# lukeshope/hipims-ocl

Hardware: AMD Instinct MI355X
Metric: Mcell-steps/sec fp64 Godunov+HLLC, 4096^2 grid, 1/2/4/8 MI355X; % HBM roofline (higher is better)
Workload: dtype f64

## Files before the change

hipims-ocl_amd/csrc/hp_engine.hip:

```cpp
#include "hp_domain.hpp"
#include "hp_observers.hpp"
#include "hp_actors.hpp"
#include <hip/hip_ext.h>
#include <dlfcn.h>

#include <algorithm>
#include <cmath>
#include <cstdio>
#include <cstdlib>
#include <cstring>
#include <random>
#include <string>
#include <vector>
#include <unistd.h>

namespace {

constexpr size_t CFL_SLOT_BYTES = 1024;

struct Rccl {
	void* handle = nullptr;
	decltype(&ncclGetUniqueId)   GetUniqueId = nullptr;
	decltype(&ncclCommInitRank)  CommInitRank = nullptr;
	decltype(&ncclCommDestroy)   CommDestroy = nullptr;
// ... 2 lines not shown
	decltype(&ncclSend)          Send = nullptr;
	decltype(&ncclRecv)          Recv = nullptr;
	decltype(&ncclAllReduce)     AllReduce = nullptr;
	decltype(&ncclGetErrorString) GetErrorString = nullptr;
	decltype(&ncclCommCount)     CommCount = nullptr;
	std::string path;
} g_rccl;

void peer_release(hp_domain* d);
PeerBox peer_box(hp_domain* d, bool use, long timeout_ms = 0);
PeerPush make_push(const hp_domain* d);

const PlanKnobs& plan_knobs()
{
	static const PlanKnobs knobs = [] {
		auto num = [](const char* name, int unset) { const char* e = std::getenv(name); return e ? std::atoi(e) : unset; };
		auto off = [&](const char* name) { return num(name, 1) == 0; };
		auto on = [&](const char* name) { return num(name, 0) != 0; };
		auto force = [&](const char* name) { return std::getenv(name) ? (num(name, 0) != 0 ? 1 : 0) : -1; };
		PlanKnobs k;
		k.two_step = num("HP_TWO_STEP", -1);
		k.launch_tail = !off("HP_LAUNCH_TAIL"); k.strip_reduce_always = on("HP_STRIP_REDUCE_ALWAYS");
		k.pair_bdy = !off("HP_PAIR_BDY"); k.pair_strict = !off("HP_PAIR_STRICT"); k.pair_exact = force("HP_PAIR_EXACT");
		k.pair_skip = !off("HP_PAIR_SKIP"); k.fill_after_pairs = !off("HP_FILL_AFTER_PAIRS");
		k.strict_speculate = on("HP_STRICT_SPECULATE"); k.pair_tune = !off("HP_PAIR_TUNE"); k.sweep_alternate = force("HP_SWEEP_ALTERNATE");
		k.tail_max_blocks = (unsigned)num("HP_TAIL_MAX_BLOCKS", (int)TAIL_MAX_BLOCKS);
		k.tail_max_blocks_k2k6 = (unsigned)num("HP_TAIL_MAX_BLOCKS_K2K6", (int)TAIL_MAX_BLOCKS);
		k.march2_rseg_forced = std::getenv("HP_MARCH2_RSEG") != nullptr;
		k.fuse_bdy = !off("HP_FUSE_BDY");
		return k;
	}();
	return knobs;
}
PlanDomain plan_domain(const hp_domain* d)
{
	PlanDomain p;
	p.scheme = d->desc.scheme; p.kernel = d->desc.kernel; p.math_mode = d->desc.math_mode; p.precision = d->desc.precision; p.dynamic_dt = d->desc.dynamic_dt;
	p.quirks = d->desc.quirks; p.rows = d->desc.rows; p.cols = d->desc.cols; p.cells = d->cells;
	p.row_offset = d->desc.row_offset; p.global_rows = d->desc.global_rows; p.ghost_rows = d->ghost_rows;
	p.has_bdy = !d->bdy.empty(); p.fusable = d->fusable; p.bdy_on_ring = d->bdy_on_ring;
	for (const Boundary& b : d->bdy)
		if ((b.kind == BDY_UNIFORM && b.definition == HP_UNIFORM_LOSS_RATE) || (b.kind == BDY_GRIDDED && b.definition == HP_GRIDDED_MASS_FLUX)) p.bdy_removes_water = true;
	p.has_comm = d->comm != nullptr; p.comm_world = d->comm_world; p.peer_direct = d->peer_direct; p.peer_mine = d->peer_mine != nullptr;
	p.has_tail_words = d->tail_words != nullptr; p.tail_allowed = d->tail_allowed; p.halo_overlap = d->halo_overlap; p.split_now = d->split_now;
	p.strip_any_bdy = d->strip_any_bdy; p.strip_first = d->strip_first; p.strip_any_full = d->strip_any_full;
	p.spec_now = d->spec_now; p.has_stamps = d->z_state != nullptr; p.march2_pays = d->tiling.march2_pays;
	p.has_links = d->links.groups != 0; p.soil_on = d->soil.on; p.tracer_on = d->tracer.on;
// ... 533 lines not shown
	bool in_place = false;
	if (bdy && !d->facts->m1_valid) {
		if ((rc = pair_cold_start<T>(d)) != HP_OK) return rc;
		in_place = true;
	} else if (bdy) in_place = d->facts->pair_fused_next;
	tail.pair = bdy ? 2 : 1;
	tail.bdy_flag = bdy && followed ? 1 : 0;
	PairAux<T> aux{};
	const bool exact = pair_exact(pd, knobs) && d->z_state != nullptr;
	if (exact) aux.stamps = StampBufs<T>{(char*)d->z_state, d->haz_words};
	aux.prev_gen = d->facts->other_stale ? d->pair_gen : 0u;
	aux.gen = ++d->pair_gen;
	if (aux.gen == 0) aux.gen = ++d->pair_gen;
	aux.list = (const AreaBdyList<T>*)d->fused_list; aux.fuse_next = bdy && followed ? 1 : 0; aux.in_place = in_place ? 1 : 0;
	aux.truncated = (d->desc.quirks & HP_QUIRK_BDY_TRUNCATED) != 0 ? 1 : 0;
	const bool recs = pair_records(pd, knobs, strip, exact, rseg2);
	if (recs) {
		if ((rc = still_rec_alloc(d, tm.nstrips)) != HP_OK) return rc;
		StillRec* const base = (StillRec*)d->still_rec;
		aux.still_out = base + (size_t)(d->still_rec_half ^ 1) * d->still_rec_slots;
		aux.still_in = d->facts->still_rec_valid ? base + (size_t)d->still_rec_half * d->still_rec_slots : nullptr;
		aux.still_rows = d->desc.rows;
	}
	const bool ordered = pair_order_on() && d->desc.precision == 8 && d->desc.math_mode != HP_MATH_STRICT && !strip && !bdy && !exact &&
	                     tm.groups <= (int)ORDER_MAX_GROUPS;
	bool order_read = false;
	if (ordered) {
		if ((rc = order_alloc(d, tm)) != HP_OK) return rc;
		order_read = d->order_written && d->flux_launches == d->order_launch + 1;
		const size_t table = (size_t)tm.nbands * tm.groups * (tm.nbig + tm.ntail);
		aux.order_in = order_read ? d->order_buf + (size_t)d->order_half * table : nullptr;
		aux.order_out = d->order_buf + (size_t)(d->order_half ^ 1) * table;
		aux.order_flags = d->order_buf + 2 * table;
	}
	const void* src = d->state[0];
	void* dst = d->state[1];
	const bool sample = d->timing_stride > 0 && d->timing_used < d->timing_events.size() &&
	                    (d->timing_counter++ % (uint64_t)d->timing_stride) == 0;
	if (sample) HIP_TRY(hipEventRecord(d->timing_events[d->timing_used].first, d->stream));
#define HP_LAUNCH_K1B2(CFL_, BDY_, HZ_, TAIL_)                                                                                            \
	hipLaunchKernelGGL((godunov_march2<false, CFL_, BDY_, HZ_, TAIL_, T>), dim3(blocks), dim3(256), 0, d->stream, p, (const Scalars<T>*)d->scalars, \
	                   (const T*)d->bed, (const State4<T>*)src, (State4<T>*)dst, (const T*)d->manning, (T*)d->cfl_slot,                    \
	                   (const T*)d->cfl_slot + SLOT_EDGE, tm, tail, aux)
#define HP_LAUNCH_K1B(CFL_, BDY_, TAIL_) do { if (exact) HP_LAUNCH_K1B2(CFL_, BDY_, true, TAIL_); else HP_LAUNCH_K1B2(CFL_, BDY_, false, TAIL_); } while (0)
	if (d->desc.math_mode == HP_MATH_STRICT)
		hipLaunchKernelGGL((godunov_march2<true, 1, false, true, 1, T>), dim3(blocks), dim3(256), 0, d->stream, p, (const Scalars<T>*)d->scalars,
// ... 1335 lines not shown
	d->timing_stride = enable_stride > 0 ? enable_stride : 0;
	return HP_OK;
}

int hp_kernel_timing_read(hp_domain_t* d, double* avg_ms, uint32_t* samples)
{
	int rc = check_domain(d);
	if (rc != HP_OK) return rc;
	if (!avg_ms || !samples) return fail(HP_ERR_INVALID, "null argument");
	HIP_TRY(hipStreamSynchronize(d->stream));
	double total = 0.0;
	uint32_t n = 0;
	for (size_t i = 0; i < d->timing_used; ++i) {
		float ms = 0.f;
		HIP_TRY(hipEventElapsedTime(&ms, d->timing_events[i].first, d->timing_events[i].second));
		total += std::max(0.0, (double)ms - d->timing_overhead_ms);
		++n;
	}
	*avg_ms = n ? total / n : 0.0;
	*samples = n;
	return HP_OK;
}

int hp_pair_stats(hp_domain_t* d, uint64_t out[12])
{
	int rc = check_domain(d);
	if (rc != HP_OK) return rc;
	if (!out) return fail(HP_ERR_INVALID, "out == NULL");
	out[0] = d->pairs; out[1] = d->pair_cold_starts; out[2] = out[3] = 0;
	HIP_TRY(hipStreamSynchronize(d->stream));
	if (tuner_on(plan_domain(d), plan_knobs()) && (rc = tuner_poll(d)) != HP_OK) return rc;
	out[4] = d->tune_samples; out[5] = d->tune_switches; out[6] = d->tune_prefer_pairs ? 1 : 0;
	out[7] = d->tune_single_ms > 0.f ? (uint64_t)(1000.0 * d->tune_pair_ms / d->tune_single_ms) : 0;
	out[8] = out[9] = out[10] = out[11] = 0;
	if (d->still_rec && d->still_rec_last) {
		const StillRec* half = (const StillRec*)d->still_rec + (size_t)d->still_rec_half * d->still_rec_slots;
		unsigned long long* counts = (unsigned long long*)((StillRec*)d->still_rec + 2 * d->still_rec_slots);
		HIP_TRY(hipMemsetAsync(counts, 0, 16, d->stream));
		hipLaunchKernelGGL(still_rec_count, dim3(256), dim3(256), 0, d->stream, half, d->still_rec_slots, counts);
		HIP_TRY(hipGetLastError());
		unsigned long long host_counts[2] = {0, 0};
		HIP_TRY(hipMemcpyAsync(host_counts, counts, sizeof host_counts, hipMemcpyDeviceToHost, d->stream));
		HIP_TRY(hipStreamSynchronize(d->stream));
		out[9] = host_counts[0]; out[10] = host_counts[1];
	}
	if (d->order_buf && d->order_read) {
		const unsigned per_band = (unsigned)(d->order_shape[1] * (d->order_shape[2] + d->order_shape[3])), table = (unsigned)d->order_shape[0] * per_band;
		unsigned* const count = d->order_buf + 2 * (size_t)table + (size_t)d->order_shape[0] * d->order_shape[1];
		HIP_TRY(hipMemsetAsync(count, 0, sizeof(unsigned), d->stream));
		hipLaunchKernelGGL(order_count, dim3(16), dim3(256), 0, d->stream, d->order_buf + (size_t)(d->order_half ^ 1) * table, (unsigned)d->order_shape[1],
		                   per_band, table, count);
		HIP_TRY(hipGetLastError());
		unsigned moved = 0;
		HIP_TRY(hipMemcpyAsync(&moved, count, sizeof moved, hipMemcpyDeviceToHost, d->stream));
		HIP_TRY(hipStreamSynchronize(d->stream));
		out[11] = moved;
	}
	if (d->haz_words) {
		unsigned long long used = 0;
		HIP_TRY(hipMemcpy(&used, d->haz_words + 2, sizeof used, hipMemcpyDeviceToHost));
		out[8] = used;
	}
	if (!d->z_state) return HP_OK;
	unsigned long long* counts = d->haz_words + 4;
	HIP_TRY(hipMemsetAsync(counts, 0, 16, d->stream));
	if (d->desc.precision == 8)
// ... 32 lines not shown
```

hipims-ocl_amd/csrc/hp_kernels.hpp:

```cpp
#pragma once

#include "hp_math.hpp"
#include "hp_tiling.hpp"
#include "hp_order.hpp"

namespace hp {

template <bool STRICT, typename T>
__global__ __launch_bounds__(256) void godunov_basic(const Params<T> p, const Scalars<T>* __restrict__ sc,
                                                     const T* __restrict__ bed, const State4<T>* __restrict__ src,
                                                     State4<T>* __restrict__ dst, const T* __restrict__ manning,
                                                     const long y_lo, const long y_hi)
{
	const long x = (long)blockIdx.x * blockDim.x + threadIdx.x;
	const long y = (long)blockIdx.y * blockDim.y + threadIdx.y + y_lo;
	if (x >= p.cols - 1 || y >= y_hi || x <= 0) return;
	const size_t id = (size_t)y * p.cols + x;
	const T dt = sc->dt;

	if (dt <= T(0)) { dst[id] = src[id]; return; }

	const State4<T> c = src[id];
	const T zb = bed[id], n = manning[id];
	if (c.zmax <= T(-9999.0) || c.z == T(-9999.0)) { dst[id] = c; return; }
// ... 509 lines not shown
template <typename T> struct AreaBdyList { int count; AreaBdy<T> b[AREA_BDY_MAX]; };


constexpr int FUSED_BDY_MAX = 3;
template <typename T> struct FusedBdy {
	T    inc_lo, inc_hi;
	int  y_switch;
	int  mode;
};

template <typename T> constexpr unsigned stamp_rec() { return (unsigned)sizeof(State4<T>) + 16u; }
template <typename T> struct StampBufs { char* rec; unsigned long long* haz; };
template <typename T> __device__ __forceinline__ unsigned stamp_gen(const StampBufs<T>& b, const size_t id)
{
	return *reinterpret_cast<const unsigned*>(b.rec + id * stamp_rec<T>() + sizeof(State4<T>));
}
template <typename T> __device__ __forceinline__ State4<T> stamp_state(const StampBufs<T>& b, const size_t id)
{
	const T* v = reinterpret_cast<const T*>(b.rec + id * stamp_rec<T>());
	State4<T> c; c.z = v[0]; c.zmax = v[1]; c.qx = v[2]; c.qy = v[3];
	return c;
}
struct StillRec { unsigned long long z, b; unsigned tag, pad[3]; };
constexpr unsigned STILL_TAG_RUN = 1, STILL_TAG_SKIP = 2;
template <typename T> struct PairAux {
	StampBufs<T>          stamps;
	unsigned              gen, prev_gen;
	const AreaBdyList<T>* list;
	int                   fuse_next;
	int                   in_place;
	int                   truncated;
	StillRec*             still_out;
	const StillRec*       still_in;
	long                  still_rows;
	const unsigned*       order_in;
	unsigned*             order_out;
	unsigned*             order_flags;
};

#ifndef HP_K1_STRICT_WAVES
#define HP_K1_STRICT_WAVES 3
#endif
#ifndef HP_K1_FAST_WAVES
#define HP_K1_FAST_WAVES 3
#endif
#ifndef HP_K1_F32_WAVES
#define HP_K1_F32_WAVES 5
#endif
template <bool STRICT, typename T> constexpr int march_waves() { return sizeof(T) == 4 ? HP_K1_F32_WAVES : (STRICT ? HP_K1_STRICT_WAVES : HP_K1_FAST_WAVES); }

template <bool STRICT, typename T> constexpr int march_waves_max() { return sizeof(T) == 4 ? 8 : march_waves<STRICT, T>(); }
template <bool STRICT, int CFL_MODE, bool FUSED, int TAIL, typename T, bool SPEC = false>
__global__ __launch_bounds__(256) __attribute__((amdgpu_waves_per_eu(march_waves<STRICT, T>(), march_waves_max<STRICT, T>()))) void godunov_march(const Params<T> p, const Scalars<T>* sc,
                                                     const T* __restrict__ bed, const State4<T>* __restrict__ src,
                                                     State4<T>* __restrict__ dst, const T* __restrict__ manning,
                                                     T* cfl_slot, const T* __restrict__ edge_max,
                                                     const TileMap tm, const AreaBdyList<T>* __restrict__ fused_list,
// ... 489 lines not shown
	}
	const bool fuse = BDY && aux.fuse_next != 0;

	T vmax = T(0), vmax1 = T(0);
	unsigned stale_rows = 0;

	constexpr bool RECS = !STRICT && !BDY && !HZ && TAIL == 1 && sizeof(T) == 8;
	unsigned long long still_kz = 0, still_kb = 0;
	unsigned still_marks = 0;
	auto write_recs = [&](const unsigned tag) {
		if (!RECS || aux.still_out == nullptr) return;
		const __amdgpu_buffer_rsrc_t srd = make_srd(aux.still_out + (size_t)strip * aux.still_rows, (size_t)aux.still_rows * sizeof(StillRec));
		const bool m = lane < 32 && ((still_marks >> (unsigned)lane) & 1u) != 0;
		hp_u32x4 a;
		a.x = m ? (unsigned)still_kz : ~0u; a.y = m ? (unsigned)(still_kz >> 32) : ~0u;
		a.z = m ? (unsigned)still_kb : ~0u; a.w = m ? (unsigned)(still_kb >> 32) : ~0u;
		unsigned voff = lane < y1 - y0 ? (unsigned)((y0 + lane) * (long)sizeof(StillRec)) : HP_OOB;
		asm volatile("" : "+v"(voff));
		store_operands_own(a);
		__builtin_amdgcn_raw_buffer_store_b128(a, srd, (int)voff, 0, 0);
		__builtin_amdgcn_raw_buffer_store_b32(m ? tag : 0u, srd, (int)voff + 16, 0, 0);
		store_fence(a, voff, 0u);
	};
	auto tile_known = [&]() -> bool {
		const long xw = strip * MARCH2_COLS - 1;
		if (xw < 1 || xw + 63 > p.cols - 2 || y0 - 2 < 1 || y1 + 1 > last_row - 1 || y1 - y0 > 32) return false;
		const int nr = (int)(y1 - y0) + 4, n = 3 * nr;
		const __amdgpu_buffer_rsrc_t srd = make_srd(aux.still_in + (size_t)(strip - 1) * aux.still_rows, (size_t)3 * aux.still_rows * sizeof(StillRec));
		auto voff = [&](const int i) {
			const int w = i < nr ? 0 : (i < 2 * nr ? 1 : 2);
			return i < n ? (unsigned)(((long)w * aux.still_rows + y0 - 2 + (i - w * nr)) * (long)sizeof(StillRec)) : HP_OOB;
		};
		const hp_u32x4 e0 = __builtin_amdgcn_raw_buffer_load_b128(srd, (int)voff(lane), 0, 0);
		const hp_u32x4 e1 = __builtin_amdgcn_raw_buffer_load_b128(srd, (int)voff(lane + 64), 0, 0);
		const unsigned k0 = __builtin_amdgcn_readfirstlane(e0.x), k1 = __builtin_amdgcn_readfirstlane(e0.y);
		const unsigned k2 = __builtin_amdgcn_readfirstlane(e0.z), k3 = __builtin_amdgcn_readfirstlane(e0.w);
		if (k0 == ~0u && k1 == ~0u) return false;
		auto same = [&](const hp_u32x4& e) { return e.x == k0 && e.y == k1 && e.z == k2 && e.w == k3; };
		if (!wave_all((lane >= n || same(e0)) && (lane + 64 >= n || same(e1)))) return false;
		still_kz = ((unsigned long long)k1 << 32) | k0;
		still_kb = ((unsigned long long)k3 << 32) | k2;
		return true;
	};

	auto march = [&](auto live_tag, auto look_tag) {
	constexpr bool LIVE = decltype(live_tag)::value;
	constexpr bool LOOK = decltype(look_tag)::value;
	auto apply = [&](auto j_tag, State4<T> c, const T zb, const long y) {
// ... 220 lines not shown
		rP = load_row(yb);
		{
			RowRegs<T> rs = load_row(yb - 2);
			if (live0) { rs.c = apply(J0(), rs.c, rs.zb, yb - 2 < 0 ? 0 : yb - 2); rc.c = apply(J0(), rc.c, rc.zb, yb - 1); }
			const Side<T> sS = make_side<STRICT>(rs.c.z, rs.c.qx, rs.c.qy, rs.zb, vs);
			sCa = make_side<STRICT>(rc.c.z, rc.c.qx, rc.c.qy, rc.zb, vs);
			drySa = (rs.c.z - rs.zb) < vs;
			if (STILL) {
				if (at_rest(rs.c)) stA |= REST_S;
				if (at_rest(rc.c)) stA |= REST_C;
				if (stA == (REST_S | REST_C) && same_level(rs.c, rs.zb, rc.c, rc.zb)) stA |= EQ_S;
			}
			if (!skip_a) fSa = face_solve<AXIS_Y, STRICT, true, true>(sS, sCa, vs).forR;
		}
		const T n0 = rc.n;
		uc = stage_a(yb - 1, rP, rQ);
		n_c = n0;
		sCb = make_side<STRICT>(uc.c.z, uc.c.qx, uc.c.qy, uc.zb, vs);
		if (STILL && at_rest(uc.c)) stB |= REST_C;
		const T n1 = rc.n;
		const RowU1<T> u0 = stage_a(yb, rQ, rP);
		stage_b(yb - 1, u0, n1, false);
	};
	auto still_run = [&]() -> long {
		auto load_rz = [&](const long yl) {
			unsigned vs_ = yl <= y1 + 1 ? voff_state : HP_OOB, vc_ = yl <= y1 + 1 ? voff_scalar : HP_OOB;
			asm volatile("" : "+v"(vs_), "+v"(vc_));
			const unsigned k = (unsigned)((yl < 0 ? 0 : (yl > last_row ? last_row : yl)) - row_base);
			RowRegs<T> q;
			q.c = buf_load_state(srd_src, vs_, k * row_state, T());
			q.zb = buf_load_scalar(srd_bed, vc_, k * row_scalar, T());
			return q;
		};
		long y = y0;
		RowRegs<T> q[4];
		#pragma unroll
		for (int j = 0; j < 4; ++j) q[j] = load_rz(y - 2 + j);
		const T z0 = first_lane(q[0].c.z), b0 = first_lane(q[0].zb), h0 = z0 - b0;
		if (!(h0 > vs && h0 < T(1e100) && z0 != T(-9999.0))) return y;
		const unsigned long long run_z = value_bits(z0), run_b = value_bits(b0);
		auto in_run = [&](const RowRegs<T>& q_) {
			return wave_all(value_bits(q_.c.z) == run_z && value_bits(q_.zb) == run_b && value_bits(q_.c.qx) == 0 && value_bits(q_.c.qy) == 0 &&
			                !(q_.c.zmax <= T(-9999.0))) != 0;
		};
		if (!(in_run(q[0]) && in_run(q[1]) && in_run(q[2]) && in_run(q[3]))) return y;
		const T spd = cfl_speed<STRICT>(q[2].c.z, q[2].c.zmax, q[2].c.qx, q[2].c.qy, q[2].zb, p.qs);
		still_kz = run_z; still_kb = run_b;
		auto put = [&](State4<T> c, const long yy) {
			if (RECS && !wave_any(!(c.zmax > T(-9999.0)) || (c.z > c.zmax && c.zmax > T(-9990.0)))) still_marks |= 1u << (unsigned)(yy - y0);
			if (c.z > c.zmax && c.zmax > T(-9990.0)) c.zmax = c.z;
			const unsigned row_k = (unsigned)__builtin_amdgcn_readfirstlane((int)(yy - row_base));
			buf_store_state(c, srd_dst, out_x ? voff_state : HP_OOB, row_k * row_state);
			if (TAIL == 2) store_peer(c, yy, out_x);
			if (CFL_MODE == 1 && out_x && (int)yy >= tm.price_lo && (int)yy < tm.price_hi && spd > vmax) vmax = spd;
		};
		State4<T> a = q[2].c, b = q[3].c;
		for (;;) {
			if (y >= y1) return y;
			#pragma unroll
			for (int j = 0; j < 4; ++j) q[j] = load_rz(y + 2 + j);
			if (!in_run(q[0])) return y;
			put(a, y);
			if (y + 1 >= y1 || !in_run(q[1])) return y + 1;
			put(b, y + 1);
			if (y + 2 >= y1 || !in_run(q[2])) return y + 2;
			put(q[0].c, y + 2);
			if (y + 3 >= y1 || !in_run(q[3])) return y + 3;
			put(q[1].c, y + 3);
			a = q[2].c; b = q[3].c;
			y += 4;
		}
	};

	const long yb = (RUNS && !skip_a && !skip_b) ? still_run() : y0;
	write_recs(STILL_TAG_RUN);
	if (!RUNS || yb < y1) {
		if constexpr (ORDERED) { if (order_word != nullptr && lane == 0) __hip_atomic_fetch_add(order_word, 1u, __ATOMIC_RELAXED, __HIP_MEMORY_SCOPE_AGENT); }
		prime(yb);
		long r = yb + 1;
		for (; r + 1 <= y1; r += 2) {
			{ const T nn = rc.n; const RowU1<T> u = stage_a(r, rP, rQ); stage_b(r - 1, u, nn, true); }
			{ const T nn = rc.n; const RowU1<T> u = stage_a(r + 1, rQ, rP); stage_b(r, u, nn, true); }
		}
		if (r <= y1) { const T nn = rc.n; const RowU1<T> u = stage_a(r, rP, rQ); stage_b(r - 1, u, nn, true); }
	}

	if (wave_any(stale_rows != 0)) {
		for (long y = y0; y < y1; ++y) {
			if ((stale_rows >> (unsigned)(y - y0)) & 1u) {
				const size_t id = (size_t)y * p.cols + xc;
				const T zb = bed[id];
				State4<T> c = src[id];
				if (live0) c = apply(J0(), c, zb, y);
				State4<T> next = c;
				if (live2) next = apply(J2(), c, zb, y);
				dst[id] = fuse ? next : c;
				if (TAIL == 2) store_peer(fuse ? next : c, y, true);
				if (CFL_MODE == 1 && (int)y >= tm.price_lo && (int)y < tm.price_hi) {
					const T s = cfl_speed<STRICT>(c.z, c.zmax, c.qx, c.qy, zb, p.qs);
					if (s > vmax) vmax = s;
					if (live2) {
						const T s2 = cfl_speed<STRICT>(next.z, next.zmax, next.qx, next.qy, zb, p.qs);
						if (s2 > vmax1) vmax1 = s2;
					}
				}
			}
		}
	}
	if (!live2) vmax1 = vmax;
	};

	auto raise_word = [&]() { if (hz_on && wave_any(stamped) && lane == 0) aux.stamps.haz[aux.gen & 1u] = (unsigned long long)aux.gen; };
	if (RECS && aux.still_in != nullptr && !skip_a && !skip_b && tile_known()) {
		still_marks = ~0u;
		write_recs(STILL_TAG_SKIP);
		if (CFL_MODE == 1 && out_x && (int)y1 > tm.price_lo && (int)y0 < tm.price_hi)
			vmax = cfl_speed<STRICT>(T(__longlong_as_double((long long)still_kz)), T(0), T(0), T(0), T(__longlong_as_double((long long)still_kb)), p.qs);
		vmax1 = vmax;
	} else {
	if (BDY && act != 0) { if (hz_any) march(std::true_type(), std::true_type()); else march(std::true_type(), std::false_type()); }
	else                 { if (hz_any) march(std::false_type(), std::true_type()); else march(std::false_type(), std::false_type()); }
	raise_word();
	}

	if (CFL_MODE != 0) {
		if (blockIdx.x == 0 && wave == 0) { const T e = *edge_max; if (e > vmax) vmax = e; if (e > vmax1) vmax1 = e; }
		vmax = wave_max(vmax);
		if (BDY) vmax1 = wave_max(vmax1);
		if (TAIL != 0) { wave_vmax = vmax; wave_vmax1 = vmax1; }
		else if (lane == 0 && vmax > T(0)) atomic_max_nonneg(cfl_slot, vmax);
	}
	}
	if (TAIL != 0) tail_block_done<BDY>(tail, wave_vmax, wave, lane, y0, y1, wave_vmax1);
}

template <typename T>
__global__ __launch_bounds__(256) void stamps_to_buffer(State4<T>* __restrict__ other, const StampBufs<T> b, const unsigned gen, const size_t cells)
{
	if (b.haz[gen & 1u] != (unsigned long long)gen) return;
	for (size_t id = (size_t)blockIdx.x * blockDim.x + threadIdx.x; id < cells; id += (size_t)gridDim.x * blockDim.x)
		if (stamp_gen(b, id) == gen) other[id] = stamp_state(b, id);
}

template <typename T>
__global__ __launch_bounds__(256) void stamps_count(const StampBufs<T> b, const unsigned gen, const size_t cells, unsigned long long* counts)
{
	unsigned long long last = 0, any = 0;
	for (size_t id = (size_t)blockIdx.x * blockDim.x + threadIdx.x; id < cells; id += (size_t)gridDim.x * blockDim.x) {
		const unsigned g = stamp_gen(b, id);
		last += (g != 0 && g == gen); any += (g != 0);
	}
	for (int off = 32; off > 0; off >>= 1) { last += __shfl_down(last, off); any += __shfl_down(any, off); }
	if ((threadIdx.x & 63) == 0 && (last | any)) { atomicAdd(counts, last); atomicAdd(counts + 1, any); }
}
__global__ __launch_bounds__(256) void still_rec_count(const StillRec* __restrict__ rec, const size_t n, unsigned long long* counts)
{
	unsigned long long skipped = 0, still = 0;
	for (size_t i = (size_t)blockIdx.x * blockDim.x + threadIdx.x; i < n; i += (size_t)gridDim.x * blockDim.x) {
		const unsigned tag = rec[i].tag;
		skipped += (tag == STILL_TAG_SKIP); still += (tag == STILL_TAG_SKIP || tag == STILL_TAG_RUN);
	}
	for (int off = 32; off > 0; off >>= 1) { skipped += __shfl_down(skipped, off); still += __shfl_down(still, off); }
	if ((threadIdx.x & 63) == 0 && (skipped | still)) { atomicAdd(counts, skipped); atomicAdd(counts + 1, still); }
}
__global__ __launch_bounds__(256) void order_count(const unsigned* __restrict__ table, const unsigned groups, const unsigned per_band, const unsigned n,
                                                   unsigned* count)
{
	unsigned moved = 0;
	for (unsigned i = blockIdx.x * blockDim.x + threadIdx.x; i < n; i += gridDim.x * blockDim.x) moved += !order_is_identity(groups, i % per_band, table[i]);
	for (int off = 32; off > 0; off >>= 1) moved += __shfl_down(moved, off);
	if ((threadIdx.x & 63) == 0 && moved) atomicAdd(count, moved);
}

template <typename T>
__global__ void pair_cold_start_words(T* slot)
{
	slot[SLOT_M1] = atomic_exchange_zero(slot);
	slot[SLOT_BDY] = T(1);
}

template <typename T>
__global__ __launch_bounds__(256) void rings_compare(const State4<T>* __restrict__ a, const State4<T>* __restrict__ b, const long cols, const long rows,
                                                     unsigned long long* differ)
{
	const long n = 2 * cols + 2 * (rows - 2);
	bool bad = false;
// ... 614 lines not shown
```

hipims-ocl_amd/csrc/hp_plan.hpp:

```cpp
#pragma once
#include "../../include/hipims_mi.h"
#include "hp_facts.hpp"

#include <algorithm>
#include <cstddef>
#include <cstdint>

namespace hp {
namespace {

constexpr unsigned TAIL_MAX_BLOCKS = 65536;
constexpr uint32_t SPEC_MIN = 8;

struct PlanKnobs {
	int      two_step = -1;
	bool     launch_tail = true;
	bool     strip_reduce_always = false;
	bool     pair_bdy = true;
	bool     pair_strict = true;
	int      pair_exact = -1;
	bool     pair_skip = true;
	bool     fill_after_pairs = true;
	bool     strict_speculate = false;
	bool     pair_tune = true;
	int      sweep_alternate = -1;
	unsigned tail_max_blocks = TAIL_MAX_BLOCKS;
	unsigned tail_max_blocks_k2k6 = TAIL_MAX_BLOCKS;
	bool     march2_rseg_forced = false;
	bool     fuse_bdy = true;
};

struct PlanDomain {
	int      scheme = HP_SCHEME_GODUNOV, kernel = HP_KERNEL_AUTO, math_mode = HP_MATH_FAST, precision = 8, dynamic_dt = 1;
	unsigned quirks = HP_QUIRKS_REFERENCE;
	long     rows = 0, cols = 0;
	size_t   cells = 0;
	long     row_offset = 0, global_rows = 0, ghost_rows = 1;
	bool     has_bdy = false;
	bool     fusable = false, bdy_on_ring = false;
	bool     bdy_removes_water = false;
	bool     has_comm = false;
	int      comm_world = 1;
	bool     peer_direct = false, peer_mine = false;
	bool     has_tail_words = true, tail_allowed = false, halo_overlap = false, split_now = true;
// ... 42 lines not shown
}
inline bool pair_eligible(const PlanDomain& d, const BufferFacts& facts, const PlanKnobs& k)
{
	return pairs_possible(d, k) && facts.pair_ready(d.dynamic_dt != 0);
}
inline bool strip_pairs_possible_here(const PlanDomain& d, const BufferFacts& facts, const PlanKnobs& k)
{
	return pairs_possible_common(d, k) && d.has_comm && d.comm_world > 1 && d.peer_direct && d.ghost_rows == 2 && !facts->rings_differ;
}
inline bool pair_exact(const PlanDomain& d, const PlanKnobs& k)
{
	if (d.math_mode == HP_MATH_STRICT) return true;
	if (k.pair_exact >= 0) return k.pair_exact != 0;
	return d.bdy_removes_water;
}
inline int pair_tile_rows(const PlanDomain& d, const PlanKnobs& k, const int march2_rseg)
{
	return (d.math_mode == HP_MATH_STRICT && !k.march2_rseg_forced) ? std::min(march2_rseg, 12) : march2_rseg;
}
inline bool pair_records(const PlanDomain& d, const PlanKnobs& k, const bool strip, const bool exact, const int tile_rows)
{
	return d.precision == 8 && k.pair_skip && !strip && !d.has_bdy && !exact && d.math_mode != HP_MATH_STRICT && tile_rows <= 32;
}

inline bool fill_wanted(const PlanDomain& d, const BufferFacts& facts, const PlanKnobs& k)
{
	return k.fill_after_pairs && facts->other_stale && d.scheme == HP_SCHEME_GODUNOV && d.kernel != HP_KERNEL_BASIC && !(pair_exact(d, k) && d.has_stamps);
}

inline bool spec_wanted(const PlanDomain& d, const PlanKnobs& k, const uint32_t n)
{
	const bool fusable_ok = d.spec_fused_kept || !d.fusable;
	return k.strict_speculate && n >= SPEC_MIN && d.math_mode == HP_MATH_STRICT && d.precision == 8 && !d.has_comm && fusable_ok && !d.has_links && !d.soil_on && !d.tracer_on &&
	       d.kernel != HP_KERNEL_BASIC && (d.scheme == HP_SCHEME_GODUNOV || d.scheme == HP_SCHEME_MUSCL_HANCOCK);
}
inline bool tuner_on(const PlanDomain& d, const PlanKnobs& k)
{
	return k.pair_tune && d.math_mode == HP_MATH_STRICT && k.two_step != 1;
}

inline bool strips_reduce_everyone(const PlanDomain& d, const BufferFacts& facts, const bool first_of_batch)
{
	const bool dst_is_primary = facts->use_alt == 1;
	return d.dynamic_dt && (d.scheme == HP_SCHEME_MUSCL_HANCOCK || !reads_primary(d) || dst_is_primary || basic_godunov(d) || d.strip_any_bdy ||
	                        (first_of_batch && d.strip_any_full));
}
// ... 44 lines not shown
```

hipims-ocl_amd/hipims_mi/__init__.py:

```python
from __future__ import annotations

import ctypes as C
import os
import weakref

import numpy as np

HERE = os.path.dirname(os.path.abspath(__file__))
PKG_ROOT = os.path.dirname(HERE)
LIB_PATH = os.path.join(PKG_ROOT, "lib", "libhipims_mi.so")

SCHEME_GODUNOV, SCHEME_MUSCL_HANCOCK, SCHEME_INERTIAL = 0, 1, 2
ARRAY_STATE, ARRAY_BED, ARRAY_MANNING = 0, 1, 2
QUIRK_CFL_READS_PRIMARY, QUIRK_BDY_TRUNCATED, QUIRK_MUSCL_NEIGHBOUR_Y_IS_BED, QUIRKS_REFERENCE = 1, 2, 4, 7
MATH_FAST, MATH_STRICT = 0, 1
KERNEL_AUTO, KERNEL_BASIC = 0, 1
UNIFORM_RAIN_INTENSITY, UNIFORM_LOSS_RATE = 0, 1
GRIDDED_RAIN_INTENSITY, GRIDDED_RAIN_ACCUMUL, GRIDDED_MASS_FLUX = 0, 1, 2
DEPTH_IGNORE, DEPTH_IS_FSL, DEPTH_IS_DEPTH, DEPTH_IS_CRITICAL = 0, 1, 2, 3
DISCHARGE_IGNORE, DISCHARGE_IS_DISCHARGE, DISCHARGE_IS_VELOCITY, DISCHARGE_IS_VOLUME = 0, 1, 2, 3
PTR_STATE_NEXT_SRC, PTR_STATE_OTHER, PTR_BED, PTR_MANNING, PTR_CFL_MAX, PTR_SCALARS = range(6)
(OUT_DEPTH, OUT_MAXDEPTH, OUT_FSL, OUT_MAXFSL, OUT_DISCHARGE_X, OUT_DISCHARGE_Y, OUT_VELOCITY_X, OUT_VELOCITY_Y, OUT_FROUDE,
 OUT_COUNT) = range(10)
OUT_CODES = {"depth": OUT_DEPTH, "maxdepth": OUT_MAXDEPTH, "fsl": OUT_FSL, "maxfsl": OUT_MAXFSL, "dischargex": OUT_DISCHARGE_X,
# ... 3 lines not shown
OVERVIEW_FACTOR_MAX = 4096
(PEAK_SPEED, PEAK_UNIT_DISCHARGE, PEAK_HAZARD, PEAK_ARRIVAL_TIME, PEAK_WET_DURATION, PEAK_COUNT) = range(6)
PEAK_CODES = {"peakspeed": PEAK_SPEED, "peakunitdischarge": PEAK_UNIT_DISCHARGE, "hazard": PEAK_HAZARD,
              "arrivaltime": PEAK_ARRIVAL_TIME, "wetduration": PEAK_WET_DURATION}
NO_CELL = 2 ** 64 - 1

EXPORTS = [
    "hp_abi_version", "hp_device_count", "hp_device_info", "hp_last_error", "hp_set_log_sink", "hp_domain_desc_default",
    "hp_domain_create", "hp_domain_destroy", "hp_domain_upload", "hp_domain_download", "hp_domain_upload_rows", "hp_state_save", "hp_state_restore",
    "hp_domain_derive", "hp_domain_stats", "hp_overview_shape", "hp_domain_overview", "hp_domain_sparse",
    "hp_peaks_enable", "hp_peaks_disable", "hp_peaks_reset", "hp_peaks_sample", "hp_peaks_read", "hp_peaks_info",
    "hp_probes_enable", "hp_probes_disable", "hp_probes_reset", "hp_probes_sample", "hp_probes_read", "hp_probes_info",
    "hp_zones_enable", "hp_zones_disable", "hp_zones_reset", "hp_zones_sample", "hp_zones_read", "hp_zones_info",
    "hp_bed_shape_add", "hp_bed_shapes_clear", "hp_bed_apply", "hp_bed_info",
    "hp_boundary_add_uniform", "hp_boundary_add_gridded", "hp_boundary_add_cell", "hp_boundary_add_links", "hp_links_read", "hp_links_info",
    "hp_boundary_add_infiltration", "hp_infiltration_read", "hp_infiltration_info", "hp_boundary_clear", "hp_boundaries_fused",
    "hp_tracer_enable", "hp_tracer_disable", "hp_tracer_add_source", "hp_tracer_sources_clear", "hp_tracer_read", "hp_tracer_write", "hp_tracer_info", "hp_set_target_time", "hp_set_time",
    "hp_force_timestep", "hp_reset_counters", "hp_update_timestep", "hp_step_batch", "hp_read_scalars",
    "hp_sync", "hp_is_busy", "hp_step_begin", "hp_step_end", "hp_step_needs_reduction", "hp_device_ptr", "hp_stream", "hp_set_halo_overlap",
    "hp_stream_halo", "hp_comm_load", "hp_comm_unique_id", "hp_strip_comm_init", "hp_strip_step_batch", "hp_strip_update_timestep",
    "hp_strip_comm_destroy", "hp_strip_info", "hp_strip_peer_ticket", "hp_strip_peer_connect", "hp_strip_peer_round",
    "hp_strip_peer_disconnect", "hp_timer_start",
    "hp_timer_stop", "hp_kernel_timing", "hp_kernel_timing_read", "hp_kernel_timing_overhead",
    "hp_launch_counts", "hp_pair_stats",
]


class HipimsError(RuntimeError):
    pass


LOG_SINK = C.CFUNCTYPE(None, C.c_int, C.c_char_p, C.c_void_p)
_log_sink_ref = None


def set_log_sink(callback):
    global _log_sink_ref
    lib = load_library()
    if callback is None:
        sink = C.cast(None, LOG_SINK)
    else:
        sink = LOG_SINK(lambda level, msg, _user: callback(int(level), msg.decode(errors="replace")))
    _check(lib, lib.hp_set_log_sink(sink, None), "hp_set_log_sink")
    _log_sink_ref = sink


class DeviceInfo(C.Structure):
# ... 1019 lines not shown

    def kernel_timing_read(self):
        avg, n = C.c_double(0), C.c_uint32(0)
        _check(self.lib, self.lib.hp_kernel_timing_read(self.h, C.byref(avg), C.byref(n)), "hp_kernel_timing_read")
        return avg.value, n.value

    def launch_counts(self):
        if not hasattr(self.lib, "hp_launch_counts"):
            return None
        a, b = C.c_uint64(0), C.c_uint64(0)
        _check(self.lib, self.lib.hp_launch_counts(self.h, C.byref(a), C.byref(b)), "hp_launch_counts")
        return a.value, b.value

    def pair_stats(self):
        if not hasattr(self.lib, "hp_pair_stats"):
            return None
        out = (C.c_uint64 * 12)()
        self.lib.hp_pair_stats.argtypes = [C.c_void_p, C.POINTER(C.c_uint64)]
        _check(self.lib, self.lib.hp_pair_stats(self.h, out), "hp_pair_stats")
        return dict(pairs=out[0], cold_starts=out[1], stamped_last=out[2], stamped_ever=out[3], tune_samples=out[4],
                    tune_switches=out[5], prefers_pairs=bool(out[6]), pair_over_single=out[7] / 1000.0, stale_used=out[8],
                    skipped_rows=out[9], still_rows=out[10], reordered_tiles=out[11])

    def kernel_timing_overhead(self):
        if not hasattr(self.lib, "hp_kernel_timing_overhead"):
            return 0.0
        ms = C.c_double(0)
        _check(self.lib, self.lib.hp_kernel_timing_overhead(self.h, C.byref(ms)), "hp_kernel_timing_overhead")
        return ms.value

    def depth_velocity(self, state=None, bed=None):
        state = self.download() if state is None else state
        bed = self._bed_host if bed is None else bed
        depth = np.maximum(0.0, state[..., 0].astype(np.float64) - bed.astype(np.float64))
        with np.errstate(divide="ignore", invalid="ignore"):
            u = np.where(depth > 1e-8, state[..., 2] / depth, 0.0)
            v = np.where(depth > 1e-8, state[..., 3] / depth, 0.0)
        return depth, u, v
```

include/hipims_mi.h:

```cpp
#ifndef HIPIMS_MI_H
#define HIPIMS_MI_H

#include <stddef.h>
#include <stdint.h>

#ifdef __cplusplus
extern "C" {
#endif

#define HP_ABI_VERSION 2

typedef enum {
	HP_OK              =  0,
	HP_ERR_INVALID     = -1,
	HP_ERR_NO_DEVICE   = -2,
	HP_ERR_HIP         = -3,
	HP_ERR_UNSUPPORTED = -4,
	HP_ERR_STATE       = -5
} hp_status;

enum { HP_SCHEME_GODUNOV = 0, HP_SCHEME_MUSCL_HANCOCK = 1, HP_SCHEME_INERTIAL = 2 };

enum { HP_ARRAY_STATE = 0, HP_ARRAY_BED = 1, HP_ARRAY_MANNING = 2 };

// ... 282 lines not shown
	int32_t comm_ranks;
	int32_t comm_rank;
	int32_t halo_overlap;
	int32_t ghost_rows;
	int32_t peer_max;
	int32_t peer_halo;
} hp_strip_info_t;
int hp_strip_info(hp_domain_t* d, hp_strip_info_t* out);

#define HP_PEER_TICKET_BYTES 384
int hp_strip_peer_ticket(hp_domain_t* d, void* ticket_out);
int hp_strip_peer_connect(hp_domain_t* d, const void* tickets, int count, int rank, int* active);
int hp_strip_peer_round(hp_domain_t* d, double value, double* max_out);
int hp_strip_peer_disconnect(hp_domain_t* d);

int hp_timer_start(hp_domain_t* d);
int hp_timer_stop(hp_domain_t* d, float* elapsed_ms);
int hp_kernel_timing(hp_domain_t* d, int enable_stride);
int hp_kernel_timing_read(hp_domain_t* d, double* avg_ms, uint32_t* samples);
int hp_kernel_timing_overhead(hp_domain_t* d, double* overhead_ms);
int hp_launch_counts(hp_domain_t* d, uint64_t* flux_launches, uint64_t* with_tail);

int hp_pair_stats(hp_domain_t* d, uint64_t out[12]);

#ifdef __cplusplus
}
#endif
#endif
```

Before: 125,800.

## Extend still-water run skipping to tiles touching the domain boundary ring

Before this change, still-water run detection and tile skipping in the paired march kernel were disabled for tiles near the domain edge ring. Now those tiles can qualify when the boundary ring holds a uniform dry wall state. A per-wave verification solves the HLLC faces against the wall state for both half-steps and confirms the interior cell stays exactly unchanged before treating ring-adjacent rows as still. The aim is to cut flux computation and memory traffic for edge tiles of lake-at-rest regions, at the cost of extra loads and face solves in edge tiles and more complex correctness conditions. New tags and a stats entry point count wall runs and skips.

```diff
diff --git a/hipims-ocl_amd/csrc/hp_engine.hip b/hipims-ocl_amd/csrc/hp_engine.hip
--- a/hipims-ocl_amd/csrc/hp_engine.hip
+++ b/hipims-ocl_amd/csrc/hp_engine.hip
@@ -48,7 +48,7 @@
 		k.two_step = num("HP_TWO_STEP", -1);
 		k.launch_tail = !off("HP_LAUNCH_TAIL"); k.strip_reduce_always = on("HP_STRIP_REDUCE_ALWAYS");
 		k.pair_bdy = !off("HP_PAIR_BDY"); k.pair_strict = !off("HP_PAIR_STRICT"); k.pair_exact = force("HP_PAIR_EXACT");
-		k.pair_skip = !off("HP_PAIR_SKIP"); k.fill_after_pairs = !off("HP_FILL_AFTER_PAIRS");
+		k.pair_skip = !off("HP_PAIR_SKIP"); k.pair_wall = !off("HP_PAIR_WALL"); k.fill_after_pairs = !off("HP_FILL_AFTER_PAIRS");
 		k.strict_speculate = on("HP_STRICT_SPECULATE"); k.pair_tune = !off("HP_PAIR_TUNE"); k.sweep_alternate = force("HP_SWEEP_ALTERNATE");
 		k.tail_max_blocks = (unsigned)num("HP_TAIL_MAX_BLOCKS", (int)TAIL_MAX_BLOCKS);
 		k.tail_max_blocks_k2k6 = (unsigned)num("HP_TAIL_MAX_BLOCKS_K2K6", (int)TAIL_MAX_BLOCKS);
@@ -628,6 +628,7 @@
 		aux.still_in = d->facts->still_rec_valid ? base + (size_t)d->still_rec_half * d->still_rec_slots : nullptr;
 		aux.still_rows = d->desc.rows;
 	}
+	aux.wall = pair_wall_runs(knobs, recs) ? 1 : 0;
 	const bool ordered = pair_order_on() && d->desc.precision == 8 && d->desc.math_mode != HP_MATH_STRICT && !strip && !bdy && !exact &&
 	                     tm.groups <= (int)ORDER_MAX_GROUPS;
 	bool order_read = false;
@@ -2009,6 +2010,31 @@
 	return HP_OK;
 }
 
+static int still_rec_counts(hp_domain* d, unsigned long long host_counts[4])
+{
+	std::fill(host_counts, host_counts + 4, 0ull);
+	if (!d->still_rec || !d->still_rec_last) return HP_OK;
+	const StillRec* half = (const StillRec*)d->still_rec + (size_t)d->still_rec_half * d->still_rec_slots;
+	unsigned long long* counts = (unsigned long long*)((StillRec*)d->still_rec + 2 * d->still_rec_slots);
+	HIP_TRY(hipMemsetAsync(counts, 0, 32, d->stream));
+	hipLaunchKernelGGL(still_rec_count, dim3(256), dim3(256), 0, d->stream, half, d->still_rec_slots, counts);
+	HIP_TRY(hipGetLastError());
+	HIP_TRY(hipMemcpyAsync(host_counts, counts, 4 * sizeof(unsigned long long), hipMemcpyDeviceToHost, d->stream));
+	HIP_TRY(hipStreamSynchronize(d->stream));
+	return HP_OK;
+}
+
+int hp_pair_wall_stats(hp_domain_t* d, uint64_t out[2])
+{
+	int rc = check_domain(d);
+	if (rc != HP_OK) return rc;
+	if (!out) return fail(HP_ERR_INVALID, "out == NULL");
+	unsigned long long counts[4];
+	if ((rc = still_rec_counts(d, counts)) != HP_OK) return rc;
+	out[0] = counts[2]; out[1] = counts[3];
+	return HP_OK;
+}
+
 int hp_pair_stats(hp_domain_t* d, uint64_t out[12])
 {
 	int rc = check_domain(d);
@@ -2020,15 +2046,9 @@
 	out[4] = d->tune_samples; out[5] = d->tune_switches; out[6] = d->tune_prefer_pairs ? 1 : 0;
 	out[7] = d->tune_single_ms > 0.f ? (uint64_t)(1000.0 * d->tune_pair_ms / d->tune_single_ms) : 0;
 	out[8] = out[9] = out[10] = out[11] = 0;
-	if (d->still_rec && d->still_rec_last) {
-		const StillRec* half = (const StillRec*)d->still_rec + (size_t)d->still_rec_half * d->still_rec_slots;
-		unsigned long long* counts = (unsigned long long*)((StillRec*)d->still_rec + 2 * d->still_rec_slots);
-		HIP_TRY(hipMemsetAsync(counts, 0, 16, d->stream));
-		hipLaunchKernelGGL(still_rec_count, dim3(256), dim3(256), 0, d->stream, half, d->still_rec_slots, counts);
-		HIP_TRY(hipGetLastError());
-		unsigned long long host_counts[2] = {0, 0};
-		HIP_TRY(hipMemcpyAsync(host_counts, counts, sizeof host_counts, hipMemcpyDeviceToHost, d->stream));
-		HIP_TRY(hipStreamSynchronize(d->stream));
+	{
+		unsigned long long host_counts[4];
+		if ((rc = still_rec_counts(d, host_counts)) != HP_OK) return rc;
 		out[9] = host_counts[0]; out[10] = host_counts[1];
 	}
 	if (d->order_buf && d->order_read) {
diff --git a/hipims-ocl_amd/csrc/hp_kernels.hpp b/hipims-ocl_amd/csrc/hp_kernels.hpp
--- a/hipims-ocl_amd/csrc/hp_kernels.hpp
+++ b/hipims-ocl_amd/csrc/hp_kernels.hpp
@@ -555,7 +555,7 @@
 	return c;
 }
 struct StillRec { unsigned long long z, b; unsigned tag, pad[3]; };
-constexpr unsigned STILL_TAG_RUN = 1, STILL_TAG_SKIP = 2;
+constexpr unsigned STILL_TAG_RUN = 1, STILL_TAG_SKIP = 2, STILL_TAG_WALL_RUN = 3, STILL_TAG_WALL_SKIP = 4;
 template <typename T> struct PairAux {
 	StampBufs<T>          stamps;
 	unsigned              gen, prev_gen;
@@ -566,6 +566,7 @@
 	StillRec*             still_out;
 	const StillRec*       still_in;
 	long                  still_rows;
+	int                   wall;
 	const unsigned*       order_in;
 	unsigned*             order_out;
 	unsigned*             order_flags;
@@ -1101,8 +1102,75 @@
 		__builtin_amdgcn_raw_buffer_store_b32(m ? tag : 0u, srd, (int)voff + 16, 0, 0);
 		store_fence(a, voff, 0u);
 	};
+	constexpr bool WALL = RECS;
+	const long xw = strip * MARCH2_COLS - 1;
+	const bool near_w = xw < 1, near_e = xw + 63 > p.cols - 2, near_s = y0 - 2 < 1, near_n = y1 + 1 > last_row - 1;
+	const bool near_ring = near_w || near_e || near_s || near_n;
+	unsigned long long wall_z = 0, wall_b = 0, wall_qx = 0, wall_qy = 0;
+	bool wall_ok = false;
+	if constexpr (WALL) {
+		if (aux.wall != 0 && near_ring && !skip_a && !skip_b && p.cols >= 4 && p.rows >= 4) {
+			const size_t id_s = (size_t)y0 * p.cols + (size_t)(xw + 2);
+			const State4<T> cs = src[id_s], cw = src[0];
+			const T sz = first_lane(cs.z), sb = first_lane(bed[id_s]), wz = first_lane(cw.z), wb = first_lane(bed[0]);
+			const T wqx = first_lane(cw.qx), wqy = first_lane(cw.qy);
+			const bool s_fits = (sz - sb) > vs && (sz - sb) < T(1e100) && sz != T(-9999.0) && wave_all(value_bits(cs.qx) == 0 && value_bits(cs.qy) == 0);
+			if (s_fits && (wz - wb) < vs) {
+				const int cx = lane % 3, cy = (lane / 3) % 3;
+				const Side<T> sS = make_side<STRICT>(sz, T(0), T(0), sb, vs), sW = make_side<STRICT>(wz, wqx, wqy, wb, vs);
+				auto side_of = [&](const bool wall) {
+					Side<T> o;
+					o.eta = wall ? sW.eta : sS.eta; o.zb = wall ? sW.zb : sS.zb; o.qx = wall ? sW.qx : sS.qx; o.qy = wall ? sW.qy : sS.qy;
+					o.u0 = wall ? sW.u0 : sS.u0; o.v0 = wall ? sW.v0 : sS.v0;
+					return o;
+				};
+				const FaceFlux<T> fW = face_solve<AXIS_X, STRICT, true, true>(side_of(cx == 1), sS, vs).forR;
+				const FaceFlux<T> fE = face_solve<AXIS_X, STRICT, true, true>(sS, side_of(cx == 2), vs).forL;
+				const FaceFlux<T> fS = face_solve<AXIS_Y, STRICT, true, true>(side_of(cy == 1), sS, vs).forR;
+				const FaceFlux<T> fN = face_solve<AXIS_Y, STRICT, true, true>(sS, side_of(cy == 2), vs).forL;
+				State4<T> c0; c0.z = sz; c0.zmax = sz; c0.qx = T(0); c0.qy = T(0);
+				const State4<T> ua = godunov_update_impl<STRICT, false, true>(c0, sb, T(0), dt_a, fN, fE, fS, fW, p.dx, inv_dx, vs, false, (T*)nullptr, NoProbe(), ka);
+				const State4<T> ub = godunov_update_impl<STRICT, false, true>(c0, sb, T(0), dt_b, fN, fE, fS, fW, p.dx, inv_dx, vs, false, (T*)nullptr, NoProbe(), kb);
+				auto is_s = [&](const State4<T>& u) { return value_bits(u.z) == value_bits(sz) && value_bits(u.qx) == 0 && value_bits(u.qy) == 0; };
+				const bool met = (cx == 0 || (cx == 1 ? near_w : near_e)) && (cy == 0 || (cy == 1 ? near_s : near_n));
+				wall_ok = wave_all(!met || (is_s(ua) && is_s(ub)));
+				wall_z = value_bits(wz); wall_b = value_bits(wb); wall_qx = value_bits(wqx); wall_qy = value_bits(wqy);
+				still_kz = value_bits(sz); still_kb = value_bits(sb);
+			}
+		}
+	}
+	auto wall_tile_known = [&]() -> bool {
+		if (!wall_ok || y1 - y0 > 32) return false;
+		const int nr = (int)(y1 - y0) + 4, n = 3 * nr;
+		const long w_lo = strip > 0 ? strip - 1 : 0;
+		const __amdgpu_buffer_rsrc_t srd = make_srd(aux.still_in + (size_t)w_lo * aux.still_rows, (size_t)3 * aux.still_rows * sizeof(StillRec));
+		auto wanted = [&](const int i, long& win, long& row) {
+			const int w = i < nr ? 0 : (i < 2 * nr ? 1 : 2);
+			win = strip - 1 + w; row = y0 - 2 + (i - w * nr);
+			return i < n && win >= 0 && win < tm.nstrips && row >= 1 && row <= last_row - 1;
+		};
+		auto entry_ok = [&](const int i) {
+			long win, row;
+			const bool want = wanted(i, win, row);
+			const hp_u32x4 e = __builtin_amdgcn_raw_buffer_load_b128(srd, want ? (int)(unsigned)(((win - w_lo) * aux.still_rows + row) * (long)sizeof(StillRec)) : (int)HP_OOB, 0, 0);
+			return !want || ((((unsigned long long)e.y << 32) | e.x) == still_kz && (((unsigned long long)e.w << 32) | e.z) == still_kb);
+		};
+		const bool recs_ok = entry_ok(lane) && entry_ok(lane + 64);
+		auto is_w = [&](const long row, const long col) {
+			const size_t id = (size_t)row * p.cols + (size_t)col;
+			const State4<T> c = src[id];
+			return value_bits(c.z) == wall_z && value_bits(bed[id]) == wall_b && value_bits(c.qx) == wall_qx && value_bits(c.qy) == wall_qy;
+		};
+		bool ring_ok = true;
+		const long row_l = y0 - 2 + lane < 0 ? 0 : (y0 - 2 + lane > last_row ? last_row : y0 - 2 + lane);
+		if (near_w) ring_ok = ring_ok && (lane >= nr || is_w(row_l, 0));
+		if (near_e) ring_ok = ring_ok && (lane >= nr || is_w(row_l, p.cols - 1));
+		if (near_s) ring_ok = ring_ok && is_w(0, xc);
+		if (near_n) ring_ok = ring_ok && is_w(last_row, xc);
+		return wave_all(recs_ok && ring_ok);
+	};
 	auto tile_known = [&]() -> bool {
-		const long xw = strip * MARCH2_COLS - 1;
+		if (WALL && near_ring) return wall_tile_known();
 		if (xw < 1 || xw + 63 > p.cols - 2 || y0 - 2 < 1 || y1 + 1 > last_row - 1 || y1 - y0 > 32) return false;
 		const int nr = (int)(y1 - y0) + 4, n = 3 * nr;
 		const __amdgpu_buffer_rsrc_t srd = make_srd(aux.still_in + (size_t)(strip - 1) * aux.still_rows, (size_t)3 * aux.still_rows * sizeof(StillRec));
@@ -1369,6 +1437,7 @@
 		const RowU1<T> u0 = stage_a(yb, rQ, rP);
 		stage_b(yb - 1, u0, n1, false);
 	};
+	bool wall_run = false;
 	auto still_run = [&]() -> long {
 		auto load_rz = [&](const long yl) {
 			unsigned vs_ = yl <= y1 + 1 ? voff_state : HP_OOB, vc_ = yl <= y1 + 1 ? voff_scalar : HP_OOB;
@@ -1383,18 +1452,26 @@
 		RowRegs<T> q[4];
 		#pragma unroll
 		for (int j = 0; j < 4; ++j) q[j] = load_rz(y - 2 + j);
-		const T z0 = first_lane(q[0].c.z), b0 = first_lane(q[0].zb), h0 = z0 - b0;
+		const bool walled = WALL && wall_ok;
+		const T z0 = walled ? T(__longlong_as_double((long long)still_kz)) : first_lane(q[0].c.z);
+		const T b0 = walled ? T(__longlong_as_double((long long)still_kb)) : first_lane(q[0].zb), h0 = z0 - b0;
 		if (!(h0 > vs && h0 < T(1e100) && z0 != T(-9999.0))) return y;
 		const unsigned long long run_z = value_bits(z0), run_b = value_bits(b0);
-		auto in_run = [&](const RowRegs<T>& q_) {
-			return wave_all(value_bits(q_.c.z) == run_z && value_bits(q_.zb) == run_b && value_bits(q_.c.qx) == 0 && value_bits(q_.c.qy) == 0 &&
-			                !(q_.c.zmax <= T(-9999.0))) != 0;
+		auto in_run = [&](const RowRegs<T>& q_, const long yl) {
+			const bool is_s = value_bits(q_.c.z) == run_z && value_bits(q_.zb) == run_b && value_bits(q_.c.qx) == 0 && value_bits(q_.c.qy) == 0 &&
+			                  !(q_.c.zmax <= T(-9999.0));
+			if constexpr (WALL) {
+				const bool is_w = value_bits(q_.c.z) == wall_z && value_bits(q_.zb) == wall_b && value_bits(q_.c.qx) == wall_qx && value_bits(q_.c.qy) == wall_qy;
+				const bool ring_cell = walled && (ring_x || yl <= 0 || yl >= last_row);
+				return wave_all(ring_cell ? is_w : is_s) != 0;
+			} else return wave_all(is_s) != 0;
 		};
-		if (!(in_run(q[0]) && in_run(q[1]) && in_run(q[2]) && in_run(q[3]))) return y;
+		if (!(in_run(q[0], y - 2) && in_run(q[1], y - 1) && in_run(q[2], y) && in_run(q[3], y + 1))) return y;
+		wall_run = walled;
 		const T spd = cfl_speed<STRICT>(q[2].c.z, q[2].c.zmax, q[2].c.qx, q[2].c.qy, q[2].zb, p.qs);
 		still_kz = run_z; still_kb = run_b;
 		auto put = [&](State4<T> c, const long yy) {
-			if (RECS && !wave_any(!(c.zmax > T(-9999.0)) || (c.z > c.zmax && c.zmax > T(-9990.0)))) still_marks |= 1u << (unsigned)(yy - y0);
+			if (RECS && !wave_any(!(WALL && walled && ring_x) && (!(c.zmax > T(-9999.0)) || (c.z > c.zmax && c.zmax > T(-9990.0))))) still_marks |= 1u << (unsigned)(yy - y0);
 			if (c.z > c.zmax && c.zmax > T(-9990.0)) c.zmax = c.z;
 			const unsigned row_k = (unsigned)__builtin_amdgcn_readfirstlane((int)(yy - row_base));
 			buf_store_state(c, srd_dst, out_x ? voff_state : HP_OOB, row_k * row_state);
@@ -1406,13 +1483,13 @@
 			if (y >= y1) return y;
 			#pragma unroll
 			for (int j = 0; j < 4; ++j) q[j] = load_rz(y + 2 + j);
-			if (!in_run(q[0])) return y;
+			if (!in_run(q[0], y + 2)) return y;
 			put(a, y);
-			if (y + 1 >= y1 || !in_run(q[1])) return y + 1;
+			if (y + 1 >= y1 || !in_run(q[1], y + 3)) return y + 1;
 			put(b, y + 1);
-			if (y + 2 >= y1 || !in_run(q[2])) return y + 2;
+			if (y + 2 >= y1 || !in_run(q[2], y + 4)) return y + 2;
 			put(q[0].c, y + 2);
-			if (y + 3 >= y1 || !in_run(q[3])) return y + 3;
+			if (y + 3 >= y1 || !in_run(q[3], y + 5)) return y + 3;
 			put(q[1].c, y + 3);
 			a = q[2].c; b = q[3].c;
 			y += 4;
@@ -1420,7 +1497,7 @@
 	};
 
 	const long yb = (RUNS && !skip_a && !skip_b) ? still_run() : y0;
-	write_recs(STILL_TAG_RUN);
+	write_recs(wall_run ? STILL_TAG_WALL_RUN : STILL_TAG_RUN);
 	if (!RUNS || yb < y1) {
 		if constexpr (ORDERED) { if (order_word != nullptr && lane == 0) __hip_atomic_fetch_add(order_word, 1u, __ATOMIC_RELAXED, __HIP_MEMORY_SCOPE_AGENT); }
 		prime(yb);
@@ -1460,7 +1537,7 @@
 	auto raise_word = [&]() { if (hz_on && wave_any(stamped) && lane == 0) aux.stamps.haz[aux.gen & 1u] = (unsigned long long)aux.gen; };
 	if (RECS && aux.still_in != nullptr && !skip_a && !skip_b && tile_known()) {
 		still_marks = ~0u;
-		write_recs(STILL_TAG_SKIP);
+		write_recs(WALL && near_ring ? STILL_TAG_WALL_SKIP : STILL_TAG_SKIP);
 		if (CFL_MODE == 1 && out_x && (int)y1 > tm.price_lo && (int)y0 < tm.price_hi)
 			vmax = cfl_speed<STRICT>(T(__longlong_as_double((long long)still_kz)), T(0), T(0), T(0), T(__longlong_as_double((long long)still_kb)), p.qs);
 		vmax1 = vmax;
@@ -1502,13 +1579,20 @@
 }
 __global__ __launch_bounds__(256) void still_rec_count(const StillRec* __restrict__ rec, const size_t n, unsigned long long* counts)
 {
-	unsigned long long skipped = 0, still = 0;
+	unsigned long long skipped = 0, still = 0, wall_skipped = 0, wall_still = 0;
 	for (size_t i = (size_t)blockIdx.x * blockDim.x + threadIdx.x; i < n; i += (size_t)gridDim.x * blockDim.x) {
 		const unsigned tag = rec[i].tag;
-		skipped += (tag == STILL_TAG_SKIP); still += (tag == STILL_TAG_SKIP || tag == STILL_TAG_RUN);
-	}
-	for (int off = 32; off > 0; off >>= 1) { skipped += __shfl_down(skipped, off); still += __shfl_down(still, off); }
-	if ((threadIdx.x & 63) == 0 && (skipped | still)) { atomicAdd(counts, skipped); atomicAdd(counts + 1, still); }
+		wall_skipped += (tag == STILL_TAG_WALL_SKIP); wall_still += (tag == STILL_TAG_WALL_SKIP || tag == STILL_TAG_WALL_RUN);
+		skipped += (tag == STILL_TAG_SKIP || tag == STILL_TAG_WALL_SKIP); still += (tag >= STILL_TAG_RUN && tag <= STILL_TAG_WALL_SKIP);
+	}
+	for (int off = 32; off > 0; off >>= 1) {
+		skipped += __shfl_down(skipped, off); still += __shfl_down(still, off);
+		wall_skipped += __shfl_down(wall_skipped, off); wall_still += __shfl_down(wall_still, off);
+	}
+	if ((threadIdx.x & 63) == 0 && (skipped | still)) {
+		atomicAdd(counts, skipped); atomicAdd(counts + 1, still);
+		if (wall_still) { atomicAdd(counts + 2, wall_skipped); atomicAdd(counts + 3, wall_still); }
+	}
 }
 __global__ __launch_bounds__(256) void order_count(const unsigned* __restrict__ table, const unsigned groups, const unsigned per_band, const unsigned n,
                                                    unsigned* count)
diff --git a/hipims-ocl_amd/csrc/hp_plan.hpp b/hipims-ocl_amd/csrc/hp_plan.hpp
--- a/hipims-ocl_amd/csrc/hp_plan.hpp
+++ b/hipims-ocl_amd/csrc/hp_plan.hpp
@@ -20,6 +20,7 @@
 	bool     pair_strict = true;
 	int      pair_exact = -1;
 	bool     pair_skip = true;
+	bool     pair_wall = true;
 	bool     fill_after_pairs = true;
 	bool     strict_speculate = false;
 	bool     pair_tune = true;
@@ -108,6 +109,7 @@
 {
 	return d.precision == 8 && k.pair_skip && !strip && !d.has_bdy && !exact && d.math_mode != HP_MATH_STRICT && tile_rows <= 32;
 }
+inline bool pair_wall_runs(const PlanKnobs& k, const bool records) { return records && k.pair_wall; }
 
 inline bool fill_wanted(const PlanDomain& d, const BufferFacts& facts, const PlanKnobs& k)
 {
diff --git a/hipims-ocl_amd/hipims_mi/__init__.py b/hipims-ocl_amd/hipims_mi/__init__.py
--- a/hipims-ocl_amd/hipims_mi/__init__.py
+++ b/hipims-ocl_amd/hipims_mi/__init__.py
@@ -49,7 +49,7 @@
     "hp_strip_comm_destroy", "hp_strip_info", "hp_strip_peer_ticket", "hp_strip_peer_connect", "hp_strip_peer_round",
     "hp_strip_peer_disconnect", "hp_timer_start",
     "hp_timer_stop", "hp_kernel_timing", "hp_kernel_timing_read", "hp_kernel_timing_overhead",
-    "hp_launch_counts", "hp_pair_stats",
+    "hp_launch_counts", "hp_pair_stats", "hp_pair_wall_stats",
 ]
 
 
@@ -1115,6 +1115,14 @@
                     tune_switches=out[5], prefers_pairs=bool(out[6]), pair_over_single=out[7] / 1000.0, stale_used=out[8],
                     skipped_rows=out[9], still_rows=out[10], reordered_tiles=out[11])
 
+    def pair_wall_stats(self):
+        if not hasattr(self.lib, "hp_pair_wall_stats"):
+            return None
+        out = (C.c_uint64 * 2)()
+        self.lib.hp_pair_wall_stats.argtypes = [C.c_void_p, C.POINTER(C.c_uint64)]
+        _check(self.lib, self.lib.hp_pair_wall_stats(self.h, out), "hp_pair_wall_stats")
+        return out[0], out[1]
+
     def kernel_timing_overhead(self):
         if not hasattr(self.lib, "hp_kernel_timing_overhead"):
             return 0.0
diff --git a/include/hipims_mi.h b/include/hipims_mi.h
--- a/include/hipims_mi.h
+++ b/include/hipims_mi.h
@@ -328,6 +328,7 @@
 int hp_launch_counts(hp_domain_t* d, uint64_t* flux_launches, uint64_t* with_tail);
 
 int hp_pair_stats(hp_domain_t* d, uint64_t out[12]);
+int hp_pair_wall_stats(hp_domain_t* d, uint64_t out[2]);
 
 #ifdef __cplusplus
 }
```

New measurement: 149,900, median of 6. 1.19x the previous value.
